# SamuelSchlesinger/anonymous-credit-tokens

Hardware: AMD Instinct MI355X
Metric: spend-proof verifies/sec (whole node), batch=2^20 (higher is better)
Workload: dtype u32 limbs / u64 accumulators (integer)

## Files before the change

### anonymous-credit-tokens_amd/csrc/msm.h

```cpp
#pragma once
#include "ge25519.h"

namespace act {

#ifndef ACT_FB_WBITS
#define ACT_FB_WBITS 16
#endif
constexpr int FB_WBITS = ACT_FB_WBITS;
constexpr int FB_WINDOWS = (253 + FB_WBITS - 1) / FB_WBITS;
constexpr int FB_ENTRIES = 1 << FB_WBITS;
constexpr int NIELS_WORDS = 32;
constexpr size_t FB_TABLE_WORDS = (size_t)FB_WINDOWS * FB_ENTRIES * NIELS_WORDS;

ACT_HD ge_niels niels_load(const uint32_t* p) {
  ge_niels n;
#if defined(__HIP_DEVICE_COMPILE__)
  const uint4* q = reinterpret_cast<const uint4*>(p);
  uint4 a[7];
  for (int i = 0; i < 7; i++) a[i] = q[i];
  uint32_t w[28];
  for (int i = 0; i < 7; i++) { w[4 * i] = a[i].x; w[4 * i + 1] = a[i].y; w[4 * i + 2] = a[i].z; w[4 * i + 3] = a[i].w; }
  for (int i = 0; i < FE_LIMBS; i++) { n.ypx.v[i] = w[i]; n.ymx.v[i] = w[FE_LIMBS + i]; n.xy2d.v[i] = w[2 * FE_LIMBS + i]; }
#else
  for (int i = 0; i < FE_LIMBS; i++) { n.ypx.v[i] = p[i]; n.ymx.v[i] = p[FE_LIMBS + i]; n.xy2d.v[i] = p[2 * FE_LIMBS + i]; }
#endif
  return n;
}
ACT_HD void niels_store(uint32_t* p, const ge_niels& n) {
  for (int i = 0; i < FE_LIMBS; i++) { p[i] = n.ypx.v[i]; p[FE_LIMBS + i] = n.ymx.v[i]; p[2 * FE_LIMBS + i] = n.xy2d.v[i]; }
  for (int i = 3 * FE_LIMBS; i < NIELS_WORDS; i++) p[i] = 0;
}
ACT_HD ge_niels niels_from_affine(const ge& p) {
  ge_niels n;
  n.ypx = fe_carry(fe_add(p.Y, p.X));
  n.ymx = fe_carry(fe_sub(p.Y, p.X));
  n.xy2d = fe_mul(p.T, fe_d2());
  return n;
}
constexpr int GE_WORDS = 4 * FE_LIMBS;
ACT_HD void ge_words(uint32_t w[GE_WORDS], const ge& g) {
  for (int i = 0; i < FE_LIMBS; i++) { w[i] = g.X.v[i]; w[FE_LIMBS + i] = g.Y.v[i]; w[2 * FE_LIMBS + i] = g.Z.v[i]; w[3 * FE_LIMBS + i] = g.T.v[i]; }
}
ACT_HD ge ge_of_words(const uint32_t w[GE_WORDS]) {
  ge g;
  for (int i = 0; i < FE_LIMBS; i++) { g.X.v[i] = w[i]; g.Y.v[i] = w[FE_LIMBS + i]; g.Z.v[i] = w[2 * FE_LIMBS + i]; g.T.v[i] = w[3 * FE_LIMBS + i]; }
  return g;
}
ACT_HD void ge_store(uint32_t* p, const ge& g) { ge_words(p, g); }
ACT_HD ge ge_load(const uint32_t* p) { return ge_of_words(p); }

struct FbTab { const uint32_t* p; uint32_t wbits; uint32_t id; };
ACT_HD uint32_t fb_windows(uint32_t wbits) { return (253u + wbits - 1u) / wbits; }
ACT_HD size_t fb_table_words(uint32_t wbits) { return (size_t)fb_windows(wbits) * ((size_t)1 << wbits) * NIELS_WORDS; }

ACT_HD uint32_t fb_next_digit(uint32_t w[8], uint32_t wbits) {
  uint32_t digit = w[0] & ((1u << wbits) - 1u);
  for (int i = 0; i < 7; i++) w[i] = (w[i] >> wbits) | (w[i + 1] << (32u - wbits));
  w[7] >>= wbits;
  return digit;
}
ACT_HD ge fixed_base_acc(ge acc, const FbTab& t, const sc& s) {
  fe_count_fixed_base(t.id);
  uint32_t w[8];
  for (int i = 0; i < 8; i++) w[i] = s.v[i];
  const uint32_t nw = fb_windows(t.wbits);
  const size_t entries = (size_t)1 << t.wbits;
  ge_niels cur = niels_load(t.p + (size_t)fb_next_digit(w, t.wbits) * NIELS_WORDS);
  for (uint32_t pos = 1; pos < nw; pos++) {
    ge_niels nxt = niels_load(t.p + ((size_t)pos * entries + fb_next_digit(w, t.wbits)) * NIELS_WORDS);
    acc = ge_madd(acc, cur);
    cur = nxt;
  }
  return ge_madd(acc, cur);
}

struct digit4 { bool nonzero, two, neg; };
ACT_HD digit4 next_digit4(uint32_t w[8], uint32_t& carry) {
  uint32_t v = (w[0] & 3u) + carry;
  for (int i = 0; i < 7; i++) w[i] = (w[i] >> 2) | (w[i + 1] << 30);
  w[7] >>= 2;
  digit4 d;
  carry = v >= 3u ? 1u : 0u;
  d.nonzero = (v != 0u) && (v != 4u);
  d.two = (v == 2u);
  d.neg = (v == 3u);
  return d;
}
ACT_HD ge chain_step_add(const ge& acc, const ge_cached& c1, const ge_cached& c2, const digit4& d) {
  ge_cached q;
  uint32_t m2 = fe_mask(d.two);
  q.YpX = fe_select_m(c1.YpX, c2.YpX, m2);
  q.YmX = fe_select_m(c1.YmX, c2.YmX, m2);
  q.Z = fe_select_m(c1.Z, c2.Z, m2);
  q.T2d = fe_select_m(c1.T2d, c2.T2d, m2);
  q = ge_cached_cneg(q, d.neg);
  return ge_add_cached(acc, q);
}
template <int NACC>
ACT_HD void chain(ge* acc, const ge& N, const sc* s) {
  uint32_t w[NACC][8], carry[NACC];
  for (int a = 0; a < NACC; a++) { carry[a] = 0; for (int i = 0; i < 8; i++) w[a][i] = s[a].v[i]; }
  ge P = N;
  for (int step = 0; step < 127; step++) {
    ge_cached c1 = ge_to_cached(P);
    ge Q = ge_double(P);
    ge_cached c2 = ge_to_cached(Q);
    if (step < 126) P = ge_double(Q);
#pragma unroll
    for (int a = 0; a < NACC; a++) {
      digit4 d = next_digit4(w[a], carry[a]);
      if (d.nonzero) acc[a] = chain_step_add(acc[a], c1, c2, d);
    }
  }
}

struct naf_state { uint32_t w[9]; };
ACT_HD naf_state naf_init(const sc& s) { naf_state n; for (int i = 0; i < 8; i++) n.w[i] = s.v[i]; n.w[8] = 0; return n; }
ACT_HD int naf_next(naf_state& n) {
  int d = 0;
  if (n.w[0] & 1u) {
    d = 2 - (int)(n.w[0] & 3u);
    if (d < 0) {
      uint64_t c = 1;
      for (int i = 0; i < 9; i++) { c += n.w[i]; n.w[i] = (uint32_t)c; c >>= 32; }
    } else {
      n.w[0] &= ~1u;
    }
  }
  for (int i = 0; i < 8; i++) n.w[i] = (n.w[i] >> 1) | (n.w[i + 1] << 31);
  n.w[8] >>= 1;
  return d;
}
ACT_HD int naf3_next(naf_state& n) {
  int d = 0;
  if (n.w[0] & 1u) {
    const uint32_t m = n.w[0] & 7u;
    d = m < 4u ? (int)m : (int)m - 8;
    n.w[0] &= ~7u;
    if (d < 0) {
      uint64_t c = 8;
      for (int i = 0; i < 9; i++) { c += n.w[i]; n.w[i] = (uint32_t)c; c >>= 32; }
    }
  }
  for (int i = 0; i < 8; i++) n.w[i] = (n.w[i] >> 1) | (n.w[i + 1] << 31);
  n.w[8] >>= 1;
  return d;
}
ACT_HD void chain2u(ge& acc_l, ge& acc_u, const ge& N, const sc& s_l, const sc& s_u) {
  uint32_t w[8], carry = 0;
  for (int i = 0; i < 8; i++) w[i] = s_l.v[i];
  naf_state nu = naf_init(s_u);
  ge P = N;
  for (int step = 0; step < 127; step++) {
    ge_cached c1 = ge_to_cached(P);
    ge Q = ge_double(P);
    ge_cached c2 = ge_to_cached(Q);
    if (step < 126) P = ge_double(Q);
    digit4 d = next_digit4(w, carry);
    if (d.nonzero) acc_l = chain_step_add(acc_l, c1, c2, d);
    int u0 = naf_next(nu);
    if (u0 != 0) acc_u = ge_add_cached(acc_u, ge_cached_cneg(c1, u0 < 0));
    int u1 = naf_next(nu);
    if (u1 != 0) acc_u = ge_add_cached(acc_u, ge_cached_cneg(c2, u1 < 0));
  }
}

constexpr int BUCKETS = 9;
constexpr int BUCKET_WORDS = BUCKETS * GE_WORDS;

constexpr int GE_PIECES = GE_WORDS / 4;
ACT_HD ge bucket_load(const uint32_t* p) {
#if defined(__HIP_DEVICE_COMPILE__)
  const uint4* q = reinterpret_cast<const uint4*>(p);
  uint4 a[GE_PIECES];
  for (int i = 0; i < GE_PIECES; i++) a[i] = q[i];
  uint32_t w[GE_WORDS];
  for (int i = 0; i < GE_PIECES; i++) { w[4 * i] = a[i].x; w[4 * i + 1] = a[i].y; w[4 * i + 2] = a[i].z; w[4 * i + 3] = a[i].w; }
  return ge_of_words(w);
#else
  return ge_load(p);
#endif
}
ACT_HD void bucket_store(uint32_t* p, const ge& g) {
#if defined(__HIP_DEVICE_COMPILE__)
  uint32_t w[GE_WORDS];
  ge_words(w, g);
  uint4* q = reinterpret_cast<uint4*>(p);
  for (int i = 0; i < GE_PIECES; i++) q[i] = make_uint4(w[4 * i], w[4 * i + 1], w[4 * i + 2], w[4 * i + 3]);
#else
  ge_store(p, g);
#endif
}
constexpr int GE_LDS_WORDS_PER_WAVE = GE_PIECES * 64 * 4;

#if defined(__HIP_DEVICE_COMPILE__)
__device__ __forceinline__ void ge_to_lds(uint32_t* lds_wave, const ge& g) {
  const uint32_t lane = threadIdx.x & 63u;
  uint32_t w[GE_WORDS];
  ge_words(w, g);
  for (int k = 0; k < GE_PIECES; k++)
    *reinterpret_cast<uint4*>(lds_wave + (k * 64 + lane) * 4) = make_uint4(w[4 * k], w[4 * k + 1], w[4 * k + 2], w[4 * k + 3]);
}
__device__ __forceinline__ ge ge_from_lds(const uint32_t* lds_wave) {
  const uint32_t lane = threadIdx.x & 63u;
  uint32_t w[GE_WORDS];
  for (int k = 0; k < GE_PIECES; k++) {
    const uint4 q = *reinterpret_cast<const uint4*>(lds_wave + (k * 64 + lane) * 4);
    w[4 * k] = q.x; w[4 * k + 1] = q.y; w[4 * k + 2] = q.z; w[4 * k + 3] = q.w;
  }
  return ge_of_words(w);
}
#endif

constexpr int NAF_WORDS = 64;
ACT_HD void naf3_recode(uint32_t out[NAF_WORDS], const sc& s) {
  naf_state n = naf_init(s);
  for (int step = 0; step < NAF_WORDS; step++) {
    uint32_t wd = 0;
    for (int k = 0; k < 4; k++) wd |= ((uint32_t)naf3_next(n) & 0xffu) << (8 * k);
    out[step] = wd;
  }
}
ACT_HD void radix16_bias(uint32_t t[8], const sc& s) {
  uint64_t c = 0;
  for (int i = 0; i < 8; i++) { c += (uint64_t)s.v[i] + 0x88888888u; t[i] = (uint32_t)c; c >>= 32; }
}
ACT_HD int naf_byte(uint32_t wd, int k) { return (int)(int8_t)(wd >> (8 * k)); }

template <bool UNIFORM>
ACT_HD void chain_bu_pre(ge& acc_l, ge& acc_u, const ge& N, const uint32_t* dg, const uint32_t* nafw, uint32_t* bk, uint32_t* lds_wave = nullptr, bool n_small = false) {
  const ge id = ge_identity();
  uint32_t touched = 0;
#if defined(__HIP_DEVICE_COMPILE__)
  ge_to_lds(lds_wave, id);
  ge_to_lds(lds_wave + GE_LDS_WORDS_PER_WAVE, id);
  auto add_u = [&](const ge_ded& q, int d) {
    uint32_t* home = lds_wave + ((d == 3 || d == -3) ? GE_LDS_WORDS_PER_WAVE : 0);
    ge_to_lds(home, ge_add_ded(ge_from_lds(home), ge_ded_cneg(q, d < 0)));
  };
#else
  ge U[2] = {id, id};
  auto add_u = [&](const ge_ded& q, int d) {
    ge& t = U[(d == 3 || d == -3) ? 1 : 0];
    t = ge_add_ded(t, ge_ded_cneg(q, d < 0));
  };
#endif
  ge P = N;
  uint32_t dw = 0;
#if defined(ACT_BUCKET_PREFETCH)
  ge Bpre = id;
  uint32_t nib_next = dg[0] & 15u;
#endif
  for (int step = 0; step < 64; step++) {
#if defined(ACT_BUCKET_PREFETCH)
    if ((step & 7) == 0) dw = dg[step >> 3] >> 4;
    const uint32_t nib = nib_next;
#else
    if ((step & 7) == 0) dw = dg[step >> 3];
    const uint32_t nib = dw & 15u; dw >>= 4;
#endif
    const bool neg = nib < 8u;
    const uint32_t mag = neg ? 8u - nib : nib - 8u;
    uint32_t nw = nafw[step];
#if defined(__HIP_DEVICE_COMPILE__)
    if (UNIFORM) nw = (uint32_t)__builtin_amdgcn_readfirstlane((int)nw);
#endif
    const int u = naf_byte(nw, 0), u1 = naf_byte(nw, 1), u2 = naf_byte(nw, 2), u3 = naf_byte(nw, 3);
    ge_ded c = ge_to_ded(P);
    uint32_t* slot = bk + mag * GE_WORDS;
    if (mag != 0u) {
#if defined(ACT_BUCKET_PREFETCH)
      ge B = Bpre;
#else
      ge B = id;
      if ((touched >> mag) & 1u) B = bucket_load(slot);
#endif
      touched |= 1u << mag;
      B = ge_add_ded(B, ge_ded_cneg(c, neg));
      bucket_store(slot, B);
    }
    if (u != 0) add_u(c, u);
    if (step == 63) {
      if (u1 != 0) { P = ge_double_opt(P, true); add_u(ge_to_ded(P), u1); }
      break;
    }
    P = ge_double_opt(P, u1 != 0);
    if (u1 != 0) add_u(ge_to_ded(P), u1);
    P = ge_double_opt(P, u2 != 0);
    if (u2 != 0) add_u(ge_to_ded(P), u2);
    P = ge_double_opt(P, u3 != 0);
    if (u3 != 0) add_u(ge_to_ded(P), u3);
#if defined(ACT_BUCKET_PREFETCH)
    {
      if (((step + 1) & 7) == 0) nib_next = dg[(step + 1) >> 3] & 15u; else { nib_next = dw & 15u; dw >>= 4; }
      const uint32_t mag_next = nib_next < 8u ? 8u - nib_next : nib_next - 8u;
      Bpre = id;
      if (mag_next != 0u && ((touched >> mag_next) & 1u)) Bpre = bucket_load(bk + mag_next * GE_WORDS);
    }
#endif
    P = ge_double_opt(P, true);
  }
  {
#if defined(__HIP_DEVICE_COMPILE__)
    ge U1 = ge_from_lds(lds_wave), U3 = ge_from_lds(lds_wave + GE_LDS_WORDS_PER_WAVE);
#else
    ge U1 = U[0], U3 = U[1];
#endif
    const uint32_t ms = fe_mask(n_small);
    U1 = ge_select_m(U1, id, ms); U3 = ge_select_m(U3, id, ms);
    acc_u = ge_add_cached(acc_u, ge_to_cached(U1));
    acc_u = ge_add_cached(acc_u, ge_to_cached(U3));
    acc_u = ge_add_cached(acc_u, ge_to_cached(ge_double_opt(U3, true)));
  }
  auto bucket = [&](int vv) { ge B = id; if ((touched >> vv) & 1u) B = bucket_load(bk + vv * GE_WORDS); return B; };
  ge S = bucket(8);
  ge R = S;
  for (int vv = 7; vv >= 1; vv--) {
    S = ge_add_cached(S, ge_to_cached(bucket(vv)));
    R = ge_add_cached(R, ge_to_cached(S));
  }
  acc_l = ge_select_m(R, id, fe_mask(n_small));
}

ACT_HD void chain_bu(ge& acc_l, ge& acc_u, const ge& N, const sc& s_l, const sc& s_u, uint32_t* bk, uint32_t* lds_wave = nullptr) {
  const ge id = ge_identity();
  for (int b = 0; b < BUCKETS; b++) bucket_store(bk + b * GE_WORDS, id);
  uint32_t w[8], carry = 0;
  for (int i = 0; i < 8; i++) w[i] = s_l.v[i];
  naf_state nu = naf_init(s_u);
#if defined(__HIP_DEVICE_COMPILE__)
  ge_to_lds(lds_wave, id);
  ge_to_lds(lds_wave + GE_LDS_WORDS_PER_WAVE, id);
  auto add_u = [&](const ge_cached& q, int d) {
    uint32_t* home = lds_wave + ((d == 3 || d == -3) ? GE_LDS_WORDS_PER_WAVE : 0);
    ge_to_lds(home, ge_add_cached(ge_from_lds(home), ge_cached_cneg(q, d < 0)));
  };
#else
  ge U[2] = {id, id};
  auto add_u = [&](const ge_cached& q, int d) {
    ge& t = U[(d == 3 || d == -3) ? 1 : 0];
    t = ge_add_cached(t, ge_cached_cneg(q, d < 0));
  };
#endif
  ge P = N;
  for (int step = 0; step < 64; step++) {
    uint32_t v = (w[0] & 15u) + carry;
    for (int i = 0; i < 7; i++) w[i] = (w[i] >> 4) | (w[i + 1] << 28);
    w[7] >>= 4;
    carry = v > 8u ? 1u : 0u;
    bool neg = v > 8u;
    uint32_t mag = neg ? 16u - v : v;
    ge_cached c = ge_to_cached(P);
    uint32_t* slot = bk + mag * GE_WORDS;
    ge B = bucket_load(slot);
    B = ge_add_cached(B, ge_cached_cneg(c, neg));
    bucket_store(slot, B);
    int u = naf3_next(nu);
    if (u != 0) add_u(c, u);
    int u1 = naf3_next(nu), u2 = naf3_next(nu), u3 = naf3_next(nu);
    if (step == 63) {
      if (u1 != 0) { P = ge_double_opt(P, true); add_u(ge_to_cached(P), u1); }
      break;
    }
    P = ge_double_opt(P, u1 != 0);
    if (u1 != 0) add_u(ge_to_cached(P), u1);
    P = ge_double_opt(P, u2 != 0);
    if (u2 != 0) add_u(ge_to_cached(P), u2);
    P = ge_double_opt(P, u3 != 0);
    if (u3 != 0) add_u(ge_to_cached(P), u3);
    P = ge_double_opt(P, true);
  }
  {
#if defined(__HIP_DEVICE_COMPILE__)
    const ge U1 = ge_from_lds(lds_wave), U3 = ge_from_lds(lds_wave + GE_LDS_WORDS_PER_WAVE);
#else
    const ge U1 = U[0], U3 = U[1];
#endif
    acc_u = ge_add_cached(acc_u, ge_to_cached(U1));
    acc_u = ge_add_cached(acc_u, ge_to_cached(U3));
    acc_u = ge_add_cached(acc_u, ge_to_cached(ge_double_opt(U3, true)));
  }
  ge S = bucket_load(bk + 8 * GE_WORDS);
  ge R = S;
  for (int vv = 7; vv >= 1; vv--) {
    S = ge_add_cached(S, ge_to_cached(bucket_load(bk + vv * GE_WORDS)));
    R = ge_add_cached(R, ge_to_cached(S));
  }
  acc_l = R;
}

template <int NACC>
ACT_HD void chain_b(ge* acc, const ge& N, const sc* s, uint32_t* bk) {
  const ge id = ge_identity();
  for (int b = 0; b < NACC * BUCKETS; b++) bucket_store(bk + b * GE_WORDS, id);
  uint32_t w[NACC][8], carry[NACC];
  for (int a = 0; a < NACC; a++) { carry[a] = 0; for (int i = 0; i < 8; i++) w[a][i] = s[a].v[i]; }
  ge P = N;
  for (int step = 0; step < 64; step++) {
    ge_cached c = ge_to_cached(P);
#pragma unroll
    for (int a = 0; a < NACC; a++) {
      uint32_t v = (w[a][0] & 15u) + carry[a];
      for (int i = 0; i < 7; i++) w[a][i] = (w[a][i] >> 4) | (w[a][i + 1] << 28);
      w[a][7] >>= 4;
      carry[a] = v > 8u ? 1u : 0u;
      bool neg = v > 8u;
      uint32_t mag = neg ? 16u - v : v;
      uint32_t* slot = bk + ((size_t)a * BUCKETS + mag) * GE_WORDS;
      bucket_store(slot, ge_add_cached(bucket_load(slot), ge_cached_cneg(c, neg)));
    }
    if (step == 63) break;
    P = ge_double_opt(P, false); P = ge_double_opt(P, false); P = ge_double_opt(P, false);
    P = ge_double_opt(P, true);
  }
  for (int a = 0; a < NACC; a++) {
    const uint32_t* ba = bk + (size_t)a * BUCKET_WORDS;
    ge S = bucket_load(ba + 8 * GE_WORDS);
    ge R = S;
    for (int vv = 7; vv >= 1; vv--) {
      S = ge_add_cached(S, ge_to_cached(bucket_load(ba + vv * GE_WORDS)));
      R = ge_add_cached(R, ge_to_cached(S));
    }
    acc[a] = ge_add_cached(acc[a], ge_to_cached(R));
  }
}

constexpr int CT_WINDOWS = 64, CT_ENTRIES = 8;
constexpr size_t CT_TABLE_WORDS = (size_t)CT_WINDOWS * CT_ENTRIES * NIELS_WORDS;
ACT_HD ge fixed_base_acc_ct(ge acc, const uint32_t* table, const sc& s) {
  uint32_t t[8];
  radix16_bias(t, s);
#pragma unroll 1
  for (int wd = 0; wd < 8; wd++) {
    uint32_t word = t[0];
    for (int i = 0; i < 7; i++) t[i] = t[i + 1];
#pragma unroll 1
    for (int k = 0; k < 8; k++) {
      const uint32_t nib = word & 15u; word >>= 4;
      const bool neg = nib < 8u;
      const uint32_t mag = neg ? 8u - nib : nib - 8u;
      const uint32_t* row = table + (size_t)(wd * 8 + k) * CT_ENTRIES * NIELS_WORDS;
      ge_niels q = ge_niels_identity();
      for (uint32_t e = 1; e <= (uint32_t)CT_ENTRIES; e++) {
        const ge_niels c = niels_load(row + (size_t)(e - 1) * NIELS_WORDS);
        const uint32_t m = fe_mask(e == mag);
        q.ypx = fe_select_m(q.ypx, c.ypx, m); q.ymx = fe_select_m(q.ymx, c.ymx, m); q.xy2d = fe_select_m(q.xy2d, c.xy2d, m);
      }
      acc = ge_madd(acc, ge_niels_cneg(q, neg));
    }
  }
  return acc;
}
#ifndef ACT_MF_KSTEPS
#define ACT_MF_KSTEPS 2
#endif
constexpr int MF_KSTEPS = ACT_MF_KSTEPS, MF_ENTRIES = 32 * MF_KSTEPS;
constexpr int MF_WBITS = MF_KSTEPS == 1 ? 6 : MF_KSTEPS == 2 ? 7 : 8, MF_WINDOWS = (253 + MF_WBITS - 1) / MF_WBITS;
constexpr int MF_WINDOW_BYTES = MF_KSTEPS * 4 * 2 * 32 * 16;
static_assert(MF_KSTEPS == 1 || MF_KSTEPS == 2 || MF_KSTEPS == 4, "32, 64 or 128 entries per window");
#if defined(__HIP_DEVICE_COMPILE__)
typedef int mf_v4i __attribute__((ext_vector_type(4)));
typedef int mf_v16i __attribute__((ext_vector_type(16)));
__device__ __forceinline__ mf_v4i mf_onehot16(int idx, int h) {
  const int rel = idx - 16 * h;
  const int val = (int)(1u << (8 * (rel & 3))), w = rel >> 2;
  mf_v4i b;
  b[0] = (w == 0) ? val : 0; b[1] = (w == 1) ? val : 0; b[2] = (w == 2) ? val : 0; b[3] = (w == 3) ? val : 0;
  return b;
}
__device__ __forceinline__ uint32_t mf_pack4(const mf_v16i& v, int q) {
  return __builtin_amdgcn_perm((uint32_t)v[4 * q + 1], (uint32_t)v[4 * q], 0x0c0c0400u) |
         (__builtin_amdgcn_perm((uint32_t)v[4 * q + 3], (uint32_t)v[4 * q + 2], 0x0c0c0400u) << 16);
}
__device__ __forceinline__ void mf_select(uint32_t w[27], const uint8_t* tabA, int idx) {
  const int lane = (int)(threadIdx.x & 63u), h = lane >> 5, r = lane & 31;
  const auto sw = __builtin_amdgcn_permlane32_swap((unsigned)idx, (unsigned)idx, false, false);
  mf_v4i b_lo[MF_KSTEPS], b_hi[MF_KSTEPS];
#pragma unroll
  for (int ks = 0; ks < MF_KSTEPS; ks++) { b_lo[ks] = mf_onehot16((int)sw[0] - 32 * ks, h); b_hi[ks] = mf_onehot16((int)sw[1] - 32 * ks, h); }
  const mf_v16i zero = {0, 0, 0, 0, 0, 0, 0, 0, 0, 0, 0, 0, 0, 0, 0, 0};
#pragma unroll
  for (int t = 0; t < 4; t++) {
    mf_v16i x = zero, y = zero;
#pragma unroll
    for (int ks = 0; ks < MF_KSTEPS; ks++) {
      const mf_v4i a = *reinterpret_cast<const mf_v4i*>(tabA + (((ks * 4 + t) * 2 + h) * 32 + r) * 16);
      x = __builtin_amdgcn_mfma_i32_32x32x32_i8(a, b_lo[ks], x, 0, 0, 0);
      y = __builtin_amdgcn_mfma_i32_32x32x32_i8(a, b_hi[ks], y, 0, 0, 0);
    }
    const int nq = t < 3 ? 4 : 2;
#pragma unroll
    for (int q = 0; q < nq; q++) {
      const bool need_hi = t < 3 || q == 0;
      uint32_t xw = mf_pack4(x, q), yw = mf_pack4(y, q);
      const auto s = __builtin_amdgcn_permlane32_swap(xw, yw, false, false);
      w[8 * t + 2 * q] = s[0];
      if (need_hi) w[8 * t + 2 * q + 1] = s[1];
    }
  }
}
__device__ __forceinline__ constexpr uint32_t mf_bias_word(int i) {
  uint32_t v = 0;
  for (int w = 0; w < MF_WINDOWS; w++) { const int bit = MF_WBITS * w + MF_WBITS - 1; if (bit / 32 == i) v |= 1u << (bit % 32); }
  return v;
}
__device__ __forceinline__ ge fixed_base_acc_mf(ge acc, const uint8_t* tab_mf, const sc& s) {
  uint32_t t[9];
  uint64_t c = 0;
  constexpr uint32_t bias[9] = {mf_bias_word(0), mf_bias_word(1), mf_bias_word(2), mf_bias_word(3), mf_bias_word(4), mf_bias_word(5), mf_bias_word(6), mf_bias_word(7), mf_bias_word(8)};
  for (int i = 0; i < 8; i++) { c += (uint64_t)s.v[i] + bias[i]; t[i] = (uint32_t)c; c >>= 32; }
  t[8] = (uint32_t)c + bias[8];
#pragma unroll 1
  for (int wd = 0; wd < MF_WINDOWS; wd++) {
    const int d = (int)(t[0] & ((1u << MF_WBITS) - 1u)) - (1 << (MF_WBITS - 1));
    for (int i = 0; i < 8; i++) t[i] = (t[i] >> MF_WBITS) | (t[i + 1] << (32 - MF_WBITS));
    t[8] >>= MF_WBITS;
    const bool neg = d < 0;
    const int mag = neg ? -d : d;
    uint32_t w[27];
    mf_select(w, tab_mf + (size_t)wd * MF_WINDOW_BYTES, mag - 1);
    const uint32_t one = mag == 0 ? 1u : 0u;
    ge_niels q;
    for (int i = 0; i < FE_LIMBS; i++) { q.ypx.v[i] = w[i]; q.ymx.v[i] = w[FE_LIMBS + i]; q.xy2d.v[i] = w[2 * FE_LIMBS + i]; }
    q.ypx.v[0] |= one; q.ymx.v[0] |= one;
    acc = ge_madd(acc, ge_niels_cneg(q, neg));
  }
  return acc;
}
#elif defined(__HIPCC__)
__device__ ge fixed_base_acc_mf(ge acc, const uint8_t* tab_mf, const sc& s);
#endif

template <int NACC>
ACT_HD void chain_ct(ge* acc, const ge& N, const sc* s, int steps = 127) {
  uint32_t w[NACC][8], carry[NACC];
  for (int a = 0; a < NACC; a++) { carry[a] = 0; for (int i = 0; i < 8; i++) w[a][i] = s[a].v[i]; }
  ge_cached idc; idc.YpX = fe_one(); idc.YmX = fe_one(); idc.Z = fe_one(); idc.T2d = fe_zero();
  ge P = N;
#pragma unroll 1
  for (int step = 0; step < steps; step++) {
    ge_cached c1 = ge_to_cached(P);
    ge Q = ge_double(P);
    ge_cached c2 = ge_to_cached(Q);
    if (step < steps - 1) P = ge_double(Q);
#pragma unroll
    for (int a = 0; a < NACC; a++) {
      digit4 d = next_digit4(w[a], carry[a]);
      const uint32_t m2 = fe_mask(d.two), mz = fe_mask(!d.nonzero);
      ge_cached q;
      q.YpX = fe_select_m(c1.YpX, c2.YpX, m2); q.YmX = fe_select_m(c1.YmX, c2.YmX, m2);
      q.Z = fe_select_m(c1.Z, c2.Z, m2); q.T2d = fe_select_m(c1.T2d, c2.T2d, m2);
      q = ge_cached_cneg(q, d.neg);
      q.YpX = fe_select_m(q.YpX, idc.YpX, mz); q.YmX = fe_select_m(q.YmX, idc.YmX, mz);
      q.Z = fe_select_m(q.Z, idc.Z, mz); q.T2d = fe_select_m(q.T2d, idc.T2d, mz);
      acc[a] = ge_add_cached(acc[a], q);
    }
  }
}
ACT_HD ge chain_ct_quarter(const ge& N, const sc& s, int i) {
  ge P = N;
#pragma unroll 1
  for (int d = 0; d < 64 * i; d++) P = ge_double(P);
  sc piece = sc_zero();
  piece.v[0] = s.v[2 * i]; piece.v[1] = s.v[2 * i + 1];
  ge acc[1] = {ge_identity()};
  sc sp[1] = {piece};
  chain_ct<1>(acc, P, sp, 33);
  return acc[0];
}
#if defined(ACT_CT_SECRET_TABLES)
template <int NACC> ACT_HD void chain_s(ge* acc, const ge& N, const sc* s, uint32_t*) { chain_ct<NACC>(acc, N, s); }
#else
template <int NACC> ACT_HD void chain_s(ge* acc, const ge& N, const sc* s, uint32_t* bk) { chain_b<NACC>(acc, N, s, bk); }
#endif

template <int E, typename Slot, typename Emit>
ACT_HD void dc_encode_batch(int count, Slot slot, Emit emit) {
  fe prefix[E];
  fe acc = fe_one();
#pragma unroll
  for (int i = 0; i < E; i++) {
    if (i < count) {
      uint32_t* w = slot(i);
      dc_efgh s = dc_prepare(bucket_load(w));
      ge t; t.X = s.e; t.Y = s.f; t.Z = s.g; t.T = s.h; bucket_store(w, t);
      fe eg, fh; bool z;
      fe prod = dc_product(eg, fh, z, s);
      prefix[i] = acc;
      acc = fe_mul(acc, prod);
    }
  }
  fe inv = fe_invert(acc);
#pragma unroll
  for (int i = E - 1; i >= 0; i--) {
    if (i < count) {
      ge t = bucket_load(slot(i));
      dc_efgh s; s.e = t.X; s.f = t.Y; s.g = t.Z; s.h = t.T;
      fe eg, fh; bool z;
      fe prod = dc_product(eg, fh, z, s);
      fe mine = fe_select(fe_mul(inv, prefix[i]), fe_zero(), z);
      inv = fe_mul(inv, prod);
      uint32_t enc[8];
      dc_finish(enc, s, eg, fh, mine);
      emit(i, enc);
    }
  }
}

}
```

### anonymous-credit-tokens_amd/csrc/spend_lanes.h

```cpp
#pragma once
#include "kernels.h"

namespace act {

#if defined(__HIP_DEVICE_COMPILE__) && defined(ACT_PIECES_NOINLINE)
#define ACT_PIECE __device__ __attribute__((noinline))
#else
#define ACT_PIECE ACT_HD
#endif

constexpr int ENC_BATCH = 32;

ACT_PIECE ge spend_prep_role_a(const SpendArgs& a, uint32_t p, uint32_t& flags) {
  const ProofLayout pl{a.P.L};
  const SpendTranscript st{a.P.L};
  const uint8_t* rec = a.proofs + (size_t)p * pl.bytes();
  uint8_t* el = a.tr + (size_t)p * a.tr_stride + 184;
  uint32_t wk[8], wa[8];
  load8(wk, rec + 32 * pl.k()); load8(wa, rec + 32 * pl.a_prime());
  ge A;
  if (!ristretto_decode(A, wa)) flags |= FLAG_UNDECODABLE;
  if (ristretto_is_identity(A)) flags |= FLAG_IDENTITY;
  sc k = sc_from_words(wk);
  tr_put_aligned(el + 40 * st.el_k(), k.v);
  tr_put_aligned(el + 40 * st.el_a_prime(), wa);
  sc gamma = load_sc(rec + 32 * pl.gamma()), e_bar = load_sc(rec + 32 * pl.e_bar());
  ge acc[1] = {ge_identity()};
  sc sa[1] = {sc_sub(e_bar, sc_mul(a.K.x, gamma))};
  chain_ct<1>(acc, A, sa);
  return acc[0];
}
ACT_PIECE void spend_prep_role_b(const SpendArgs& a, uint32_t p, uint32_t& flags, ge& a1b, ge& a2b) {
  const ProofLayout pl{a.P.L};
  const SpendTranscript st{a.P.L};
  const uint8_t* rec = a.proofs + (size_t)p * pl.bytes();
  uint8_t* el = a.tr + (size_t)p * a.tr_stride + 184;
  uint32_t wb[8];
  load8(wb, rec + 32 * pl.b_bar());
  ge B;
  if (!ristretto_decode(B, wb)) flags |= FLAG_UNDECODABLE;
  tr_put_aligned(el + 40 * st.el_b_bar(), wb);
  ge acc[2] = {ge_identity(), ge_identity()};
  sc sb[2] = {load_sc(rec + 32 * pl.r2_bar()), load_sc(rec + 32 * pl.r3_bar())};
  chain_b<2>(acc, B, sb, a.pbk + ((size_t)p * PREP_BUCKET_SETS + 1) * BUCKET_WORDS);
  a1b = acc[0]; a2b = acc[1];
}
ACT_PIECE ge spend_prep_role_c_a2(const SpendArgs& a, uint32_t p) {
  const ProofLayout pl{a.P.L};
  const uint8_t* rec = a.proofs + (size_t)p * pl.bytes();
  tr_put_prefix(a.tr + (size_t)p * a.tr_stride, a.P, LABEL_SPEND);
  sc k = load_sc(rec + 32 * pl.k()), gamma = load_sc(rec + 32 * pl.gamma());
  sc c_bar = load_sc(rec + 32 * pl.c_bar()), r_bar = load_sc(rec + 32 * pl.r_bar());
  sc ngamma = sc_neg(gamma);
  ge f = fixed_base_acc(ge_identity(), a.P.tab[BASE_H1], c_bar);
  f = fixed_base_acc(f, a.P.tab[BASE_H3], r_bar);
  f = fixed_base_acc(f, a.P.tab[BASE_G], ngamma);
  return fixed_base_acc(f, a.P.tab[BASE_H2], sc_mul(ngamma, k));
}
ACT_PIECE void spend_prep_role_c_bits(const SpendArgs& a, uint32_t p) {
  const ProofLayout pl{a.P.L};
  const uint8_t* rec = a.proofs + (size_t)p * pl.bytes();
  sc gamma = load_sc(rec + 32 * pl.gamma());
  sc w00 = load_sc(rec + 32 * pl.w00()), w01 = load_sc(rec + 32 * pl.w01());
  ge d0 = fixed_base_acc(ge_identity(), a.P.tab[BASE_H2], sc_half(w00));
  ge d1 = fixed_base_acc(ge_identity(), a.P.tab[BASE_H2], sc_half(w01));
  ge_store(a.d01 + (size_t)p * 2 * GE_WORDS, d0);
  ge_store(a.d01 + (size_t)p * 2 * GE_WORDS + GE_WORDS, d1);
  naf3_recode(a.naf + (size_t)p * NAF_WORDS, sc_half(gamma));
}
ACT_PIECE ge spend_prep_role_c(const SpendArgs& a, uint32_t p) {
  ge f = spend_prep_role_c_a2(a, p);
  spend_prep_role_c_bits(a, p);
  return f;
}
ACT_PIECE void spend_prep_put(const SpendArgs& a, uint32_t p, int element, const ge& pt) {
  uint32_t enc[8];
  ristretto_encode(enc, pt);
  tr_put_aligned(a.tr + (size_t)p * a.tr_stride + 184 + 40 * element, enc);
}
ACT_HD void spend_prep_lane(const SpendArgs& a, uint32_t p) {
  const SpendTranscript st{a.P.L};
  uint32_t flags = 0;
  ge a1a = spend_prep_role_a(a, p, flags);
  ge a1b, a2b;
  spend_prep_role_b(a, p, flags, a1b, a2b);
  ge a2f = spend_prep_role_c(a, p);
  spend_prep_put(a, p, st.el_a1(), ge_add(a1a, a1b));
  spend_prep_put(a, p, st.el_a2(), ge_add(a2f, a2b));
  a.flags[p] = flags;
}

ACT_HD void spend_prep_a_lane(const SpendArgs& a, uint32_t p) {
  uint32_t flags = 0;
  ge_store(a.part + ((size_t)p * PART_POINTS + 0) * GE_WORDS, spend_prep_role_a(a, p, flags));
  if (flags) ACT_FLAG_OR(a.flags + p, flags);
}
ACT_HD void spend_prep_b_lane(const SpendArgs& a, uint32_t p) {
  uint32_t flags = 0;
  ge a1b, a2b;
  spend_prep_role_b(a, p, flags, a1b, a2b);
  ge_store(a.part + ((size_t)p * PART_POINTS + 1) * GE_WORDS, a1b);
  ge_store(a.part + ((size_t)p * PART_POINTS + 2) * GE_WORDS, a2b);
  if (flags) ACT_FLAG_OR(a.flags + p, flags);
}
ACT_HD void spend_prep_c_lane(const SpendArgs& a, uint32_t p) {
  ge_store(a.part + ((size_t)p * PART_POINTS + 3) * GE_WORDS, spend_prep_role_c(a, p));
}
ACT_HD void spend_prep_c1_lane(const SpendArgs& a, uint32_t p) { spend_prep_role_c_bits(a, p); }
ACT_HD void spend_prep_c2_lane(const SpendArgs& a, uint32_t p) {
  ge_store(a.part + ((size_t)p * PART_POINTS + 3) * GE_WORDS, spend_prep_role_c_a2(a, p));
}
ACT_HD void spend_prep_join_lane(const SpendArgs& a, uint32_t p) {
  const SpendTranscript st{a.P.L};
  const uint32_t* q = a.part + (size_t)p * PART_POINTS * GE_WORDS;
  spend_prep_put(a, p, st.el_a1(), ge_add(ge_load(q), ge_load(q + GE_WORDS)));
  spend_prep_put(a, p, st.el_a2(), ge_add(ge_load(q + 3 * GE_WORDS), ge_load(q + 2 * GE_WORDS)));
}
ACT_HD void spend_coords_lane(const SpendArgs& a, uint32_t gid) {
  const int L = a.P.L;
  uint32_t p = gid / (uint32_t)L, j = gid % (uint32_t)L;
  if (p >= a.n) return;
  const ProofLayout pl{L};
  uint32_t wc[8];
  load8(wc, a.proofs + (size_t)p * pl.bytes() + 32 * pl.com(j));
  ge C;
  if (!ristretto_decode(C, wc)) ACT_FLAG_OR(a.flags + p, FLAG_UNDECODABLE);
  niels_store(a.coords + ((size_t)p * L + j) * NIELS_WORDS, niels_from_affine(C));
}

template <bool UNIFORM>
ACT_HD void spend_bits_lane(const SpendArgs& a, uint32_t gid, uint32_t* lds_wave) {
  const int L = a.P.L;
  uint32_t p = gid / (uint32_t)L, j = gid % (uint32_t)L;
  if (p >= a.n) return;
  const ProofLayout pl{L};
  const SpendTranscript st{L};
  const uint8_t* rec = a.proofs + (size_t)p * pl.bytes();
  uint8_t* el = a.tr + (size_t)p * a.tr_stride + 184;

  uint32_t wc[8];
  load8(wc, rec + 32 * pl.com(j));
  ge C;
  bool ok = ristretto_decode(C, wc);
  if (!ok) ACT_FLAG_OR(a.flags + p, FLAG_UNDECODABLE);
  tr_put_aligned(el + 40 * st.el_com(j), wc);
  niels_store(a.coords + ((size_t)p * L + j) * NIELS_WORDS, niels_from_affine(C));

  sc gamma = sc_half(load_sc(rec + 32 * pl.gamma()));
  sc g0 = sc_half(load_sc(rec + 32 * pl.gamma0(j)));
  sc g1 = sc_sub(gamma, g0);
  sc z0 = sc_half(load_sc(rec + 32 * pl.z(j, 0))), z1 = sc_half(load_sc(rec + 32 * pl.z(j, 1)));

  ge acc_u = fixed_base_acc(ge_identity(), a.P.tab[BASE_H3], z1);
  acc_u = fixed_base_acc(acc_u, a.P.tab[BASE_H1], g1);
  if (j == 0) acc_u = ge_add(acc_u, ge_load(a.d01 + (size_t)p * 2 * GE_WORDS + GE_WORDS));
  ge acc_l = ge_identity();
#if defined(ACT_ABLATE_BUCKET_FOOTPRINT)
  uint32_t* bk = a.buckets + (size_t)(gid % ACT_ABLATE_BUCKET_FOOTPRINT) * BUCKET_WORDS;
#else
  uint32_t* bk = a.buckets + (size_t)gid * BUCKET_WORDS;
#endif
  uint32_t* dg = a.dig + (size_t)gid * 8;
  { uint32_t t[8]; radix16_bias(t, g0); for (int i = 0; i < 8; i++) dg[i] = t[i]; }
  const bool n_small = !ok || (wc[0] | wc[1] | wc[2] | wc[3] | wc[4] | wc[5] | wc[6] | wc[7]) == 0u;
  chain_bu_pre<UNIFORM>(acc_l, acc_u, ge_neg(C), dg, a.naf + (size_t)p * NAF_WORDS, bk, lds_wave, n_small);
  ge f0 = fixed_base_acc(ge_identity(), a.P.tab[BASE_H3], z0);
  if (j == 0) f0 = ge_add(f0, ge_load(a.d01 + (size_t)p * 2 * GE_WORDS));
  ge_cached dl = ge_to_cached(acc_l);
  bucket_store(bk, ge_add_cached(f0, dl));
  bucket_store(bk + GE_WORDS, ge_add_cached(acc_u, ge_cached_cneg(dl, true)));
}

constexpr int ENC_BATCH_SMALL = 8;
template <int E>
ACT_HD void spend_enc_lane_e(const SpendArgs& a, uint64_t q0) {
  const uint32_t L = (uint32_t)a.P.L;
  const uint64_t total = (uint64_t)a.n * L * 2u;
  if (q0 >= total) return;
  const int count = (int)(total - q0 < (uint64_t)E ? total - q0 : (uint64_t)E);
  const SpendTranscript st{a.P.L};
  dc_encode_batch<E>(
      count,
      [&](int i) { uint64_t q = q0 + (uint64_t)i; return a.buckets + (size_t)(q >> 1) * BUCKET_WORDS + (q & 1u) * GE_WORDS; },
      [&](int i, const uint32_t* enc) {
        uint64_t q = q0 + (uint64_t)i, lane = q >> 1;
        uint32_t p = (uint32_t)(lane / L), j = (uint32_t)(lane % L);
        tr_put_aligned(a.tr + (size_t)p * a.tr_stride + 184 + 40 * st.el_cprime(j, (int)(q & 1u)), enc);
      });
}
ACT_HD void spend_enc_lane(const SpendArgs& a, uint64_t q0) { spend_enc_lane_e<ENC_BATCH>(a, q0); }

ACT_HD ge spend_tail_horner(const SpendArgs& a, uint32_t p, int j_lo, int j_hi, int shift) {
  const int L = a.P.L;
  ge kp = ge_identity();
  for (int j = j_hi - 1; j >= j_lo; j--) {
    kp = ge_double(kp);
    kp = ge_madd(kp, niels_load(a.coords + ((size_t)p * L + j) * NIELS_WORDS));
  }
  for (int i = 0; i < shift; i++) kp = ge_double(kp);
  return kp;
}
ACT_HD ge spend_tail_fixed(const SpendArgs& a, uint32_t p) {
  const ProofLayout pl{a.P.L};
  const uint8_t* rec = a.proofs + (size_t)p * pl.bytes();
  sc gamma = load_sc(rec + 32 * pl.gamma());
  sc s = load_sc(rec + 32 * pl.s()), c_bar = load_sc(rec + 32 * pl.c_bar());
  sc k_bar = load_sc(rec + 32 * pl.k_bar()), s_bar = load_sc(rec + 32 * pl.s_bar());
  ge f = fixed_base_acc(ge_identity(), a.P.tab[BASE_H1], sc_sub(sc_mul(sc_neg(gamma), s), c_bar));
  f = fixed_base_acc(f, a.P.tab[BASE_H2], k_bar);
  return fixed_base_acc(f, a.P.tab[BASE_H3], s_bar);
}
ACT_HD void spend_tail_c(const SpendArgs& a, uint32_t p, const ge& kp, const ge& f) {
  const ProofLayout pl{a.P.L};
  const SpendTranscript st{a.P.L};
  ge acc[1] = {f};
  sc sk_[1] = {sc_neg(load_sc(a.proofs + (size_t)p * pl.bytes() + 32 * pl.gamma()))};
  chain_b<1>(acc, kp, sk_, a.pbk + (size_t)p * PREP_BUCKET_SETS * BUCKET_WORDS);
  uint32_t enc[8];
  ristretto_encode(enc, acc[0]); tr_put_aligned(a.tr + (size_t)p * a.tr_stride + 184 + 40 * st.el_c(), enc);
}
ACT_HD void spend_tail_xa(const SpendArgs& a, uint32_t p, const ge& kp) {
  ge_store(a.xa + (size_t)p * GE_WORDS, ge_add(kp, ge_basepoint()));
  if (a.kprime_enc) { uint32_t enc[8]; ristretto_encode(enc, kp); store8(a.kprime_enc + (size_t)p * 32, enc); }
}
ACT_HD void spend_tail_lane(const SpendArgs& a, uint32_t p) {
  ge kp = spend_tail_horner(a, p, 0, a.P.L, 0);
  spend_tail_c(a, p, kp, spend_tail_fixed(a, p));
  spend_tail_xa(a, p, kp);
}
ACT_HD void spend_tail_k_lane(const SpendArgs& a, uint32_t p) { spend_tail_xa(a, p, spend_tail_horner(a, p, 0, a.P.L, 0)); }
ACT_HD void spend_tail_c_lane(const SpendArgs& a, uint32_t p) {
  const ge kp = ge_add(ge_load(a.xa + (size_t)p * GE_WORDS), ge_neg(ge_basepoint()));
  spend_tail_c(a, p, kp, spend_tail_fixed(a, p));
}

ACT_HD void spend_finish_lane(const SpendArgs& a, uint32_t p) {
  const ProofLayout pl{a.P.L};
  sc gamma = load_sc(a.proofs + (size_t)p * pl.bytes() + 32 * pl.gamma());
  uint32_t w[16];
  for (int i = 0; i < 16; i++) w[i] = a.xof[(size_t)p * 16 + i];
  sc chal = sc_from_wide_words(w);
  uint32_t f = a.flags[p];
  uint8_t stt = 0;
  if (f & FLAG_UNDECODABLE) stt = 255;
  else if (f & FLAG_IDENTITY) stt = 6;
  else if (!sc_equal(chal, gamma)) stt = 7;
  a.status[p] = stt;
  if (a.kprime_enc && stt != 0) zero8(a.kprime_enc + (size_t)p * 32);
}

}
```

Measured before the change: 529,000.

## Pick lightest NAF3 recoding among scalar candidates and fold fixed-base sums into chain

```diff
diff --git a/anonymous-credit-tokens_amd/csrc/msm.h b/anonymous-credit-tokens_amd/csrc/msm.h
--- a/anonymous-credit-tokens_amd/csrc/msm.h
+++ b/anonymous-credit-tokens_amd/csrc/msm.h
@@ -221,14 +221,77 @@
     out[step] = wd;
   }
 }
+constexpr int NAF3_TOP = 252;
+constexpr int NAF3_CANDIDATES = 8;
+ACT_HD naf_state naf3_candidate(const sc& s, int c) {
+  naf_state n; n.w[8] = 0;
+  uint32_t l[9];
+  for (int i = 0; i < 8; i++) l[i] = sc_l_word(i);
+  l[8] = 0;
+  if (c < 4) { for (int i = 0; i < 8; i++) n.w[i] = s.v[i]; } else { bn_sub<8>(n.w, l, s.v); }
+  for (int k = 0; k < (c & 3); k++) bn_add<9>(n.w, n.w, l);
+  return n;
+}
+template <typename OnDigit>
+ACT_HD bool naf3_scan(const naf_state& n, OnDigit on_digit) {
+  uint32_t carry = 0;
+  int pos = 0;
+#pragma unroll
+  for (int j = 0; j < 9; j++) {
+    const uint64_t cur = (uint64_t)n.w[j] | ((uint64_t)(j < 8 ? n.w[j + 1] : 0u) << 32);
+    while (pos < 32 * (j + 1)) {
+      const uint32_t u = ((uint32_t)(cur >> (pos & 31)) & 7u) + carry;
+      if ((u & 1u) == 0u) {
+        carry = carry & ((uint32_t)(cur >> (pos & 31)) & 1u);
+        pos += 1;
+      } else {
+        const int d = u < 4u ? (int)u : (int)u - 8;
+        if (pos > NAF3_TOP) return false;
+        on_digit(pos, d);
+        carry = d < 0 ? 1u : 0u;
+        pos += 3;
+      }
+    }
+  }
+  return carry == 0u;
+}
+ACT_HD uint32_t naf3_cost(const naf_state& n) {
+  uint32_t c = 0;
+  const bool ok = naf3_scan(n, [&](int pos, int) { c += (pos & 3) ? 9u : 8u; });
+  return ok ? c : ~0u;
+}
+ACT_HD int naf3_recode_lightest(uint32_t out[NAF_WORDS], const sc& s) {
+#if defined(ACT_NAF_PLAIN)
+  naf3_recode(out, s);
+  return 0;
+#else
+  int best = 0;
+  uint32_t best_cost = naf3_cost(naf3_candidate(s, 0));
+  for (int c = 1; c < NAF3_CANDIDATES; c++) {
+    const uint32_t cost = naf3_cost(naf3_candidate(s, c));
+    if (cost < best_cost) { best_cost = cost; best = c; }
+  }
+  if (best_cost == ~0u) { naf3_recode(out, s); return 0; }
+  const bool neg = best >= 4;
+  for (int step = 0; step < NAF_WORDS; step++) out[step] = 0;
+  int step = 0;
+  uint32_t wd = 0;
+  naf3_scan(naf3_candidate(s, best), [&](int pos, int d) {
+    if ((pos >> 2) != step) { out[step] = wd; step = pos >> 2; wd = 0; }
+    wd |= ((uint32_t)(neg ? -d : d) & 0xffu) << (8 * (pos & 3));
+  });
+  out[step] = wd;
+  return best;
+#endif
+}
 ACT_HD void radix16_bias(uint32_t t[8], const sc& s) {
   uint64_t c = 0;
   for (int i = 0; i < 8; i++) { c += (uint64_t)s.v[i] + 0x88888888u; t[i] = (uint32_t)c; c >>= 32; }
 }
 ACT_HD int naf_byte(uint32_t wd, int k) { return (int)(int8_t)(wd >> (8 * k)); }
 
-template <bool UNIFORM>
-ACT_HD void chain_bu_pre(ge& acc_l, ge& acc_u, const ge& N, const uint32_t* dg, const uint32_t* nafw, uint32_t* bk, uint32_t* lds_wave = nullptr, bool n_small = false) {
+template <bool UNIFORM, typename Fold>
+ACT_HD void chain_bu_pre_fold(ge& acc_l, const ge& N, const uint32_t* dg, const uint32_t* nafw, uint32_t* bk, uint32_t* lds_wave, bool n_small, Fold fold) {
   const ge id = ge_identity();
   uint32_t touched = 0;
 #if defined(__HIP_DEVICE_COMPILE__)
@@ -308,9 +371,7 @@
 #endif
     const uint32_t ms = fe_mask(n_small);
     U1 = ge_select_m(U1, id, ms); U3 = ge_select_m(U3, id, ms);
-    acc_u = ge_add_cached(acc_u, ge_to_cached(U1));
-    acc_u = ge_add_cached(acc_u, ge_to_cached(U3));
-    acc_u = ge_add_cached(acc_u, ge_to_cached(ge_double_opt(U3, true)));
+    fold(U1, U3);
   }
   auto bucket = [&](int vv) { ge B = id; if ((touched >> vv) & 1u) B = bucket_load(bk + vv * GE_WORDS); return B; };
   ge S = bucket(8);
@@ -320,6 +381,14 @@
     R = ge_add_cached(R, ge_to_cached(S));
   }
   acc_l = ge_select_m(R, id, fe_mask(n_small));
+}
+template <bool UNIFORM>
+ACT_HD void chain_bu_pre(ge& acc_l, ge& acc_u, const ge& N, const uint32_t* dg, const uint32_t* nafw, uint32_t* bk, uint32_t* lds_wave = nullptr, bool n_small = false) {
+  chain_bu_pre_fold<UNIFORM>(acc_l, N, dg, nafw, bk, lds_wave, n_small, [&](const ge& U1, const ge& U3) {
+    acc_u = ge_add_cached(acc_u, ge_to_cached(U1));
+    acc_u = ge_add_cached(acc_u, ge_to_cached(U3));
+    acc_u = ge_add_cached(acc_u, ge_to_cached(ge_double_opt(U3, true)));
+  });
 }
 
 ACT_HD void chain_bu(ge& acc_l, ge& acc_u, const ge& N, const sc& s_l, const sc& s_u, uint32_t* bk, uint32_t* lds_wave = nullptr) {
diff --git a/anonymous-credit-tokens_amd/csrc/spend_lanes.h b/anonymous-credit-tokens_amd/csrc/spend_lanes.h
--- a/anonymous-credit-tokens_amd/csrc/spend_lanes.h
+++ b/anonymous-credit-tokens_amd/csrc/spend_lanes.h
@@ -66,7 +66,7 @@
   ge d1 = fixed_base_acc(ge_identity(), a.P.tab[BASE_H2], sc_half(w01));
   ge_store(a.d01 + (size_t)p * 2 * GE_WORDS, d0);
   ge_store(a.d01 + (size_t)p * 2 * GE_WORDS + GE_WORDS, d1);
-  naf3_recode(a.naf + (size_t)p * NAF_WORDS, sc_half(gamma));
+  naf3_recode_lightest(a.naf + (size_t)p * NAF_WORDS, sc_half(gamma));
 }
 ACT_PIECE ge spend_prep_role_c(const SpendArgs& a, uint32_t p) {
   ge f = spend_prep_role_c_a2(a, p);
@@ -146,15 +146,19 @@
   tr_put_aligned(el + 40 * st.el_com(j), wc);
   niels_store(a.coords + ((size_t)p * L + j) * NIELS_WORDS, niels_from_affine(C));
 
+#if defined(ACT_BITS_SEPARATE_SUMS)
   sc gamma = sc_half(load_sc(rec + 32 * pl.gamma()));
+#endif
   sc g0 = sc_half(load_sc(rec + 32 * pl.gamma0(j)));
+
+#if defined(ACT_BITS_SEPARATE_SUMS)
   sc g1 = sc_sub(gamma, g0);
   sc z0 = sc_half(load_sc(rec + 32 * pl.z(j, 0))), z1 = sc_half(load_sc(rec + 32 * pl.z(j, 1)));
-
   ge acc_u = fixed_base_acc(ge_identity(), a.P.tab[BASE_H3], z1);
   acc_u = fixed_base_acc(acc_u, a.P.tab[BASE_H1], g1);
   if (j == 0) acc_u = ge_add(acc_u, ge_load(a.d01 + (size_t)p * 2 * GE_WORDS + GE_WORDS));
   ge acc_l = ge_identity();
+#endif
 #if defined(ACT_ABLATE_BUCKET_FOOTPRINT)
   uint32_t* bk = a.buckets + (size_t)(gid % ACT_ABLATE_BUCKET_FOOTPRINT) * BUCKET_WORDS;
 #else
@@ -163,12 +167,28 @@
   uint32_t* dg = a.dig + (size_t)gid * 8;
   { uint32_t t[8]; radix16_bias(t, g0); for (int i = 0; i < 8; i++) dg[i] = t[i]; }
   const bool n_small = !ok || (wc[0] | wc[1] | wc[2] | wc[3] | wc[4] | wc[5] | wc[6] | wc[7]) == 0u;
+#if defined(ACT_BITS_SEPARATE_SUMS)
   chain_bu_pre<UNIFORM>(acc_l, acc_u, ge_neg(C), dg, a.naf + (size_t)p * NAF_WORDS, bk, lds_wave, n_small);
   ge f0 = fixed_base_acc(ge_identity(), a.P.tab[BASE_H3], z0);
   if (j == 0) f0 = ge_add(f0, ge_load(a.d01 + (size_t)p * 2 * GE_WORDS));
   ge_cached dl = ge_to_cached(acc_l);
   bucket_store(bk, ge_add_cached(f0, dl));
   bucket_store(bk + GE_WORDS, ge_add_cached(acc_u, ge_cached_cneg(dl, true)));
+#else
+  ge acc_l, acc_u;
+  chain_bu_pre_fold<UNIFORM>(acc_l, ge_neg(C), dg, a.naf + (size_t)p * NAF_WORDS, bk, lds_wave, n_small, [&](const ge& U1, const ge& U3) {
+    const sc g1h = sc_sub(sc_half(load_sc(rec + 32 * pl.gamma())), sc_half(load_sc(rec + 32 * pl.gamma0(j))));
+    acc_u = fixed_base_acc(U1, a.P.tab[BASE_H3], sc_half(load_sc(rec + 32 * pl.z(j, 1))));
+    acc_u = fixed_base_acc(acc_u, a.P.tab[BASE_H1], g1h);
+    acc_u = ge_add_cached(acc_u, ge_to_cached(U3));
+    acc_u = ge_add_cached(acc_u, ge_to_cached(ge_double_opt(U3, true)));
+  });
+  if (j == 0) acc_u = ge_add(acc_u, ge_load(a.d01 + (size_t)p * 2 * GE_WORDS + GE_WORDS));
+  bucket_store(bk + GE_WORDS, ge_add_cached(acc_u, ge_cached_cneg(ge_to_cached(acc_l), true)));
+  ge f0 = fixed_base_acc(acc_l, a.P.tab[BASE_H3], sc_half(load_sc(rec + 32 * pl.z(j, 0))));
+  if (j == 0) f0 = ge_add(f0, ge_load(a.d01 + (size_t)p * 2 * GE_WORDS));
+  bucket_store(bk, f0);
+#endif
 }
 
 constexpr int ENC_BATCH_SMALL = 8;
```

After: 534,000, median of 6. No clear change (+0.9%).
